# onecodex/needletail

Hardware: AMD Instinct MI355X
Metric: Gbases/s canonical k=21 on 150 bp FASTQ; % HBM-read roofline at 1/2/4/8 GPU (higher is better)
Workload: dtype u64; 1 GPU; configs[1]: synthetic FASTQ 10M x 150 bp, k=21 canonical k-mers (normalize -> reverse_complement -> canonical_kmers), reduce mode, device-resident batch; reads_total=10000000, reads_this_gpu=10000000, read_len=150, k=21, seed=0x5eed0002, outputs=n_total,n_fwd,n_rc,4096-bin prefix histogram,sum64,xor64, parallelism=single GPU, rccl_ranks=0, devices_visible=1

## Files before the change

### needletail_amd/csrc/ntk_api.hip

```cpp
#include "../../include/needletail_amd.h"

#include <hip/hip_runtime.h>
#include <rccl/rccl.h>
#include <dlfcn.h>
#include <time.h>

#include <cstdlib>
#include <cstring>
#include <map>
#include <mutex>
#include <new>
#include <utility>
#include <thread>
#include <algorithm>
#include <vector>

#include "ntk_kernels.hpp"

using namespace ntk;

const void *ntk_pick_scan2(int k, bool tie_rc, bool accept_u);
const void *ntk_pick_scan2_q(int k, bool canonical, bool tie_rc, bool accept_u);
const void *ntk_pick_scan2_min_a(int k, int w, bool tie_rc, bool accept_u, bool quality);
const void *ntk_pick_scan2_min_b(int k, int w, bool tie_rc, bool accept_u, bool quality);
const void *ntk_pick_scan2_fwd(int k, bool accept_u);

namespace {

thread_local int g_last_hip = 0;
thread_local int g_last_rccl = 0;

inline unsigned grid_for(uint64_t items, unsigned block) { const uint64_t b = (items + block - 1) / block; return (unsigned)(b > (1u << 20) ? (1u << 20) : (b ? b : 1)); }

#define HIPCHK(expr)                                     \
    do {                                                 \
        hipError_t e__ = (expr);                         \
        if (e__ != hipSuccess) {                         \
            g_last_hip = (int)e__;                       \
            (void)hipGetLastError();                     \
            return NTK_ERR_HIP;                          \
// ... 132 lines not shown
}

struct Mode { int kw; bool canon, tie_rc, accept_u; bool raw_bytes = false; };
inline uint32_t quality_cutoff(const ntk_params *p) { return (p->flags >> 8) & 0xFFu; }

int resolve_mode(const ntk_params *p, bool batch_face, Mode *m)
{
    if (!p) return NTK_ERR_BAD_ARG;
    if (p->k < 1 || p->k > (batch_face && p->path == NTK_PATH_BYTES_CANONICAL ? 255u : 32u)) return NTK_ERR_BAD_K;
    if ((p->flags & ~(0xFFFFu | NTK_FLAG_RESET)) != 0 || p->pre > NTK_PRE_NORMALIZE_IUPAC) return NTK_ERR_BAD_ARG;
    m->kw = p->k > 16 ? 2 : 1;
    m->accept_u = p->pre >= NTK_PRE_NORMALIZE;
    switch (p->path) {
    case NTK_PATH_BYTES_CANONICAL:
        m->raw_bytes = batch_face && (p->pre < NTK_PRE_NORMALIZE || p->k > 32);
        m->canon = true; m->tie_rc = true; break;
    case NTK_PATH_BITS: m->canon = false; m->tie_rc = false; break;
    case NTK_PATH_BITS_CANONICAL: m->canon = true; m->tie_rc = false; break;
    default: return NTK_ERR_BAD_ARG;
    }
    return NTK_OK;
}

constexpr int kMaxShards = 256;
constexpr uint32_t kLowerRing = 64;
constexpr uint64_t kMaxTilesPerLaunch = (uint64_t)8 << 22;

template <bool QM>
const void *pick_materialise(const Mode &m, uint32_t k)
{
#define NTK_PICK_FIX(KF, T, U)                                                                      \
    if (!QM && m.kw == 2 && m.canon && k == KF && m.tie_rc == T && m.accept_u == U)                  \
        return (const void *)&scan_kernel<2, true, T, U, false, KF>;
    NTK_PICK_FIX(21, false, false) NTK_PICK_FIX(21, false, true) NTK_PICK_FIX(21, true, true)
#undef NTK_PICK_FIX
#define NTK_PICK(KW, C, T, U)                                                                       \
    if (m.kw == KW && m.canon == C && m.tie_rc == T && m.accept_u == U)                             \
        return (const void *)&scan_kernel<KW, C, T, U, false, 0, QM>;
    NTK_PICK(1, false, false, false) NTK_PICK(1, false, false, true)
    NTK_PICK(1, true, false, false) NTK_PICK(1, true, false, true)
    NTK_PICK(1, true, true, true)
    NTK_PICK(2, false, false, false) NTK_PICK(2, false, false, true)
    NTK_PICK(2, true, false, false) NTK_PICK(2, true, false, true)
    NTK_PICK(2, true, true, true)
#undef NTK_PICK
    return nullptr;
}

const void *pick_scan(const Mode &m, uint32_t k, bool reduce, bool quality)
// ... 130 lines not shown
    if (rc) return rc;
    Fold fold;
    fold.undigested = wide;
    TimedSpan span;
    if ((rc = span.begin(c))) return rc;
    if (packed_first) {
        const FlagPair f = next_flag(c);
        launch_with_quality(c, normalized ? wide_reduce_q<true> : wide_reduce_q<false>,
                            normalized ? &wide_canonical_reduce_kernel<true> : &wide_canonical_reduce_kernel<false>, blocks, kWkThreads, d_qual, cutoff,
                            d_seq, n, p->k, c->d_part_hist, c->d_part_scalars, f.flag, f.next);
        HIPCHK(hipGetLastError());
        fold.alt_flag = f.flag; fold.alt_rows = blocks_raw;
    }
    launch_raw_bytes(c, wide, blocks_raw, d_seq, n, p->k, fold.alt_flag, normalized, d_qual, cutoff);
    HIPCHK(hipGetLastError());
    if ((rc = span.end(c->ev_used))) return rc;
    return launch_fold(c, blocks, fold);
}

struct TileScan {
    const void *fn = nullptr;
    int threads = 0;
    size_t lds = 0;
    uint32_t halo_lanes = 0;
    uint64_t max_chunk = 0;
    int max_per_cu = 0;
    bool reduce = true;
    bool speculate = false;
    uint32_t cutoff = 0;
};
inline uint64_t tile_count(uint64_t n, uint64_t tile_slots) { return ((n + 15) / 16 + tile_slots - 1) / tile_slots; }
int launch_tile_scan(ntk_ctx *c, const TileScan &s, ScanArgs &a, bool zero_first)
{
    int per_cu = 0, rc = resident_blocks(c, s.fn, s.threads, s.lds, s.max_per_cu, &per_cu);
    if (rc) return rc;
    const uint64_t blocks_max = block_cap(c, per_cu), waves_per_block = (uint64_t)s.threads / 64;
    const uint64_t tile_slots = 64 - (uint64_t)s.halo_lanes, tile_stride = tile_slots * 16, n = a.n_bytes;
    const int blocks_raw = s.speculate ? raw_bytes_blocks(c, n) : 0;
    a.n_tiles = tile_count(n, tile_slots);
    a.work_counters = c->d_work;
    a.zero_words = NTK_ACC_WORDS;
    for (uint64_t tb = 0; tb < a.n_tiles; tb += kMaxTilesPerLaunch) {
        const uint64_t te = tb + kMaxTilesPerLaunch < a.n_tiles ? tb + kMaxTilesPerLaunch : a.n_tiles;
        const uint64_t tiles = te - tb;
        uint64_t chunk = tiles / (blocks_max * waves_per_block * 4);
        chunk = chunk < 1 ? 1 : (chunk > s.max_chunk ? s.max_chunk : chunk);
        const uint64_t want_blocks = (tiles + chunk * waves_per_block - 1) / (chunk * waves_per_block);
        const int blocks = (int)(want_blocks < blocks_max ? want_blocks : blocks_max);
        a.tile_begin = tb; a.tile_end = te;
        const uint64_t first_tail = n / tile_stride;
        a.tail_tile_rel = first_tail < tb ? 0u : (first_tail - tb > 0xFFFFFFFEull ? 0xFFFFFFFFu : (uint32_t)(first_tail - tb));
        a.n_shards = blocks < kMaxShards ? (uint32_t)blocks : (uint32_t)kMaxShards;
        a.tiles_per_shard = (uint32_t)((tiles + a.n_shards - 1) / a.n_shards);
        a.chunk_tiles = (uint32_t)chunk;
        a.zero_acc = zero_first ? c->d_acc : nullptr;
        zero_first = false;
        if (c->work_dirty) HIPCHK(hipMemsetAsync(c->d_work, 0, kMaxShards * 64, c->stream));
        c->work_dirty = true;
        if (s.reduce) {
            if ((rc = ensure_partials(c, blocks > blocks_raw ? blocks : blocks_raw))) return rc;
            a.part_hist = c->d_part_hist; a.part_scalars = c->d_part_scalars;
        }
        Fold fold;
        fold.rearm_shards = a.n_shards;
        if (s.speculate) {
            const FlagPair f = next_flag(c);
            a.lower_flag = f.flag; a.lower_flag_next = f.next;
            fold.alt_flag = f.flag; fold.alt_rows = blocks_raw;
        }
        TimedSpan span;
        if ((rc = span.begin(c))) return rc;
        void *kargs[] = {(void *)&a};
        HIPCHK(hipLaunchKernel(s.fn, dim3(blocks), dim3(s.threads), kargs, s.lds, c->stream));
        if (s.speculate) {
            launch_raw_bytes(c, false, blocks_raw, a.seq, n, a.k, fold.alt_flag, false, a.qual, s.cutoff);
            HIPCHK(hipGetLastError());
        }
        if ((rc = span.end(c->ev_used))) return rc;
        if (s.reduce && (rc = launch_fold(c, blocks, fold))) return rc;
    }
    return NTK_OK;
}

int run_scan(ntk_ctx *c, const uint8_t *d_seq, uint64_t n, const ntk_params *p, const Mode &m, bool reduce,
             uint64_t *d_values, uint16_t *d_valid16, uint16_t *d_rc16, const uint8_t *d_qual = nullptr, const void *fused_min_fn = nullptr,
             int halo_lanes = kHaloLanes)
{
    const bool zero_first = reduce && (p->flags & NTK_FLAG_RESET);
    if (n == 0) {
        if (zero_first) HIPCHK(hipMemsetAsync(c->d_acc, 0, NTK_ACC_WORDS * sizeof(uint64_t), c->stream));
        return NTK_OK;
    }
    if (bad_device_input(d_seq, d_qual)) return NTK_ERR_BAD_ARG;
    const uint32_t cutoff = d_qual ? quality_cutoff(p) : 0u;
    bool speculate = false;
    if (m.raw_bytes) {
        if (p->k > 32 && (!reduce || fused_min_fn)) return NTK_ERR_BAD_K;
        if (!reduce || fused_min_fn) return NTK_ERR_UNSUPPORTED;
        const uint8_t *qual = cutoff ? d_qual : nullptr;
        speculate = p->k <= 32 && tile_count(n, 64 - (uint64_t)halo_lanes) <= kMaxTilesPerLaunch && !(c->route_off & NTK_ROUTE_NO_SPECULATION);
        if (!speculate) return run_bytes_reduce(c, d_seq, n, p, zero_first, m.accept_u, qual, cutoff);
    }
    const void *fn = fused_min_fn ? fused_min_fn : pick_scan(m, p->k, reduce, cutoff != 0);
    if (!fn) return NTK_ERR_BAD_ARG;
    int threads = !reduce ? 256 : (c->launch_threads ? c->launch_threads : 768);
    if (reduce && !c->launch_threads) {
        auto it = c->auto_threads.find(fn);
        if (it != c->auto_threads.end()) threads = it->second;
        else {
            int best_waves = 0;
            for (int t : {768, 640, 512}) {
                int blocks_cu = 0;
                HIPCHK(hipOccupancyMaxActiveBlocksPerMultiprocessor(&blocks_cu, fn, t, 0));
                if (blocks_cu > 2) blocks_cu = 2;
                if (blocks_cu * t > best_waves) { best_waves = blocks_cu * t; threads = t; }
            }
            c->auto_threads[fn] = threads;
        }
    }
    TileScan s;
    s.fn = fn; s.threads = threads; s.halo_lanes = (uint32_t)halo_lanes; s.max_chunk = 24;
    s.lds = reduce ? 0 : (size_t)(threads / 64) * kStageWaveU64 * sizeof(uint64_t);
    s.max_per_cu = reduce ? 2 * (1024 / threads) : 4;
    s.reduce = reduce; s.speculate = speculate; s.cutoff = cutoff;
    ScanArgs a;
    memset(&a, 0, sizeof(a));
    scan_args_set_k(a, p->k);
    a.seq = d_seq; a.n_bytes = n;
    a.values = d_values; a.valid16 = d_valid16; a.rc16 = d_rc16;
    scan_args_set_quality(a, d_qual, cutoff);
    return launch_tile_scan(c, s, a, zero_first);
}

const void *pick_min_generic(const Mode &m, bool quality, bool f64, uint32_t k)
{
    const int kw = f64 ? 2 : m.kw;
    const int mode = min_gen_mode(k, f64);
#define NTK_PICK_MG(KW, T, U, Q, F, MD) if (kw == KW && m.tie_rc == T && m.accept_u == U && quality == Q && f64 == F && mode == MD) return (const void *)&minimizer_scan_kernel<KW, T, U, Q, F, MD>;
#define NTK_PICK_MG3(KW, Q, F, MD) NTK_PICK_MG(KW, false, false, Q, F, MD) NTK_PICK_MG(KW, false, true, Q, F, MD) NTK_PICK_MG(KW, true, true, Q, F, MD)
#define NTK_PICK_MG6(KW, F, MD) NTK_PICK_MG3(KW, false, F, MD) NTK_PICK_MG3(KW, true, F, MD)
    NTK_PICK_MG6(2, true, 0) NTK_PICK_MG6(2, true, 1) NTK_PICK_MG6(2, true, 3) NTK_PICK_MG6(2, true, 2)
    NTK_PICK_MG6(2, false, 2)
    NTK_PICK_MG6(2, false, 1) NTK_PICK_MG6(1, false, 0) NTK_PICK_MG6(1, false, 1)
#undef NTK_PICK_MG6
#undef NTK_PICK_MG3
#undef NTK_PICK_MG
    return nullptr;
}

int run_min_scan(ntk_ctx *c, const uint8_t *d_seq, uint64_t n, const ntk_params *p, const Mode &m, uint32_t w, const uint8_t *d_qual)
{
    if (bad_device_input(d_seq, d_qual)) return NTK_ERR_BAD_ARG;
    const uint32_t cutoff = d_qual ? quality_cutoff(p) : 0u;
    const bool f64 = p->k <= 25 && !(c->route_off & NTK_ROUTE_NO_F64);
    ScanArgs a;
    memset(&a, 0, sizeof(a));
    scan_args_set_k(a, p->k);
    a.seq = d_seq; a.n_bytes = n;
    scan_args_set_quality(a, d_qual, cutoff);
    scan_args_set_window(a, w);
    TileScan s;
    s.fn = pick_min_generic(m, cutoff != 0, f64, p->k);
    if (!s.fn) return NTK_ERR_BAD_ARG;
    s.threads = min_gen_threads(f64);
    s.halo_lanes = a.min_halo_lanes; s.max_chunk = 16; s.max_per_cu = 8;
    return launch_tile_scan(c, s, a, (p->flags & NTK_FLAG_RESET) != 0);
}

void destroy_batch(ntk_batch *b)
{
    if (b->h_seq) (void)hipHostFree(b->h_seq);
    if (b->h_off) (void)hipHostFree(b->h_off);
    if (b->d_seq) (void)hipFree(b->d_seq);
    if (b->h_qual) (void)hipHostFree(b->h_qual);
    if (b->d_qual) (void)hipFree(b->d_qual);
    if (b->ev_copied) (void)hipEventDestroy(b->ev_copied);
    if (b->ev_done) (void)hipEventDestroy(b->ev_done);
    delete b;
}

int init_ctx(ntk_ctx *c, void *stream, bool borrow);

int create_ctx(int device, void *stream, bool borrow, ntk_ctx **out)
{
    if (!out) return NTK_ERR_BAD_ARG;
    *out = nullptr;
    int count = 0;
    if (hipGetDeviceCount(&count) != hipSuccess || count <= 0) { (void)hipGetLastError(); return NTK_ERR_NO_DEVICE; }
// ... 1019 lines not shown
}


static int minimizers_reduce_impl(ntk_ctx *c, const uint8_t *d_seq, const uint8_t *d_qual, uint64_t n, const ntk_params *p, uint32_t w);

int ntk_minimizers_reduce_device(ntk_ctx *c, const uint8_t *d_seq, uint64_t n, const ntk_params *p, uint32_t w)
{
    return minimizers_reduce_impl(c, d_seq, nullptr, n, p, w);
}

static int minimizers_reduce_impl(ntk_ctx *c, const uint8_t *d_seq, const uint8_t *d_qual, uint64_t n, const ntk_params *p, uint32_t w)
{
    if (!c || w < 1 || w > 256) return NTK_ERR_BAD_ARG;
    Mode m;
    int rc = resolve_mode(p, true, &m);
    if (rc) return rc;
    if (!m.canon) return NTK_ERR_BAD_ARG;
    if (m.raw_bytes) return p->k > 32 ? NTK_ERR_BAD_K : NTK_ERR_UNSUPPORTED;
    HIPCHK(hipSetDevice(c->device));
    if (n) {
        const bool masked = d_qual && quality_cutoff(p);
        const void *fn = (c->route_off & NTK_ROUTE_NO_REGFUSED) ? nullptr : pick_scan_min(m, p->k, w, masked);
        if (fn)
            return run_scan(c, d_seq, n, p, m, true, nullptr, nullptr, nullptr, masked ? d_qual : nullptr, fn, p->k + w - 1 > 32 ? 3 : 2);
        if (p->k <= 31 && w <= 49 && !(c->route_off & NTK_ROUTE_NO_GENERIC))
            return run_min_scan(c, d_seq, n, p, m, w, masked ? d_qual : nullptr);
    }
    if (p->flags & NTK_FLAG_RESET) HIPCHK(hipMemsetAsync(c->d_acc, 0, NTK_ACC_WORDS * sizeof(uint64_t), c->stream));
    if (n == 0) return NTK_OK;
    const uint64_t chunk = c->minimizer_chunk;
    const uint64_t back = (uint64_t)w + p->k - 2;
    const int blocks = c->n_cu * 4;
    if ((rc = ensure_partials(c, blocks))) return rc;
    ScanArgs a; memset(&a, 0, sizeof(a)); scan_args_set_k(a, p->k);
    for (uint64_t c0 = 0; c0 < n; c0 += chunk) {
        const uint64_t c1 = c0 + chunk < n ? c0 + chunk : n;
        const uint64_t start = c0 > back ? (c0 - back) & ~(uint64_t)15 : 0;
        const uint64_t n_sub = c1 - start, nt = (n_sub + 15) / 16 * 16;
        if ((rc = ensure_scratch(c, 3, nt * 8))) return rc;
        if ((rc = ensure_scratch(c, 4, nt / 8 + 16))) return rc;
        if ((rc = ensure_scratch(c, 5, nt / 8 + 16))) return rc;
        uint64_t *d_val = (uint64_t *)c->scratch[3].p;
        uint16_t *d_v16 = (uint16_t *)c->scratch[4].p, *d_r16 = (uint16_t *)c->scratch[5].p;
        if ((rc = run_scan(c, d_seq + start, n_sub, p, m, false, d_val, d_v16, d_r16, d_qual ? d_qual + start : nullptr))) return rc;
#define NTK_WM(WW)                                                                                                    \
    case WW:                                                                                                          \
        hipLaunchKernelGGL(window_min_reduce_kernel<WW>, dim3(blocks), dim3(kWmThreads), 0, c->stream, (const uint64_t *)d_val, \
// ... 318 lines not shown
```

### needletail_amd/csrc/ntk_kernels.hpp

```cpp
#pragma once
#include <hip/hip_runtime.h>
#include <stdint.h>
#include <type_traits>

#include "ntk_tile.hpp"

#if !defined(NTK_KBENCH) && (defined(NTK_ABL_LOADSONLY) || defined(NTK_ABL_FLOOR) || defined(NTK_ABL_NOLDS) || defined(NTK_ABL_NODIGEST) || \
                             defined(NTK_ABL_NOEXEC) || defined(NTK_ABL_NOSDWA) || defined(NTK_ABL_NOMASKALG) || defined(NTK_V_CLOCKS) || \
                             defined(NTK_X_CMPFIRST) || defined(NTK_X_TWOPHASE) || defined(NTK_X_MFMASUM) || defined(NTK_X_SELOUT) || defined(NTK_X_PREFETCH2) || defined(NTK_X_FASTSTART) || defined(NTK_ABL_HALFIMPORTS))
#error "NTK_ABL_* / NTK_X_* / NTK_V_CLOCKS are kernel-bench switches: build with -DNTK_KBENCH (tools/build_kbench.sh), never into the library"
#endif

namespace ntk {

typedef uint32_t u32x4 __attribute__((ext_vector_type(4)));

constexpr int kDppWaveShr1 = 0x138;
struct DevXL {
    __device__ __forceinline__ uint32_t prev_and(int s, uint32_t x, uint32_t mask) const { return prev(s, x) & mask; }
    __device__ __forceinline__ uint32_t prev_auto(uint32_t x) const { return prev(0, x); }
    __device__ __forceinline__ uint32_t prev(int, uint32_t x) const
    {
        return (uint32_t)__builtin_amdgcn_mov_dpp((int)x, kDppWaveShr1, 0xf, 0xf, true);
    }
    __device__ __forceinline__ uint32_t prev_add(int, uint32_t x, uint32_t c) const
    {
        uint32_t r;
        asm("s_nop 1\n v_add_u32_dpp %0, %1, %2 wave_shr:1 row_mask:0xf bank_mask:0xf bound_ctrl:1" : "=v"(r) : "v"(x), "v"(c));
        return r;
    }
    __device__ __forceinline__ uint32_t select_prev(int, bool take, uint32_t a, uint32_t b) const
    {
// ... 175 lines not shown
            uint64_t *ps = a.part_scalars + (size_t)blockIdx.x * 4;
            ps[0] = tv; ps[1] = tf; ps[2] = ts; ps[3] = tx;
        }
    }
}

template <int K, int HB>
struct DevMasks2 {
    static constexpr bool kLight = Sv2Light<K, HB>::value;
    uint64_t VA[16], VB[16];
    uint64_t sum = 0, sum2 = 0;
    uint32_t sumh = 0;
    uint32_t xh = 0, xlo = 0;
    uint32_t rep = 0;
    static constexpr int kWordCopies = K <= 6 ? (((1 << HB) >> (2 * (K <= 6 ? K : 0))) < 64 ? ((1 << HB) >> (2 * (K <= 6 ? K : 0))) : 64) : 1;
    uint32_t one = 1;
    uint32_t nf_s = 0;
    uint32_t nf_bits = 0;
#ifdef NTK_X_MFMASUM
    typedef int i32x4 __attribute__((ext_vector_type(4)));
    i32x4 macc = {0, 0, 0, 0}, msel = {0, 0, 0, 0};
#endif

    template <int KM, class Enc>
    __device__ __forceinline__ void compute(const Enc &en, bool tail_tile, int64_t lane_base, uint64_t n_bytes)
    {
        uint64_t B[16];
#ifdef NTK_X_CLEANTILE
        {
            const uint32_t dif = (en.ex[0] ^ en.uu[0]) | (en.ex[1] ^ en.uu[1]) | (en.ex[2] ^ en.uu[2]) | (en.ex[3] ^ en.uu[3]);
            if (!tail_tile && __builtin_amdgcn_ballot_w64(dif != 0u) == 0ull) {
#pragma unroll
                for (int i = 0; i < 16; i++) { VA[i] = Sv2Geom<KM>::kKeep; VB[i] = ~0ull; }
                asm volatile("" ::: "memory");
                return;
            }
        }
#endif
#ifdef NTK_ABL_NOSDWA
#pragma unroll
        for (int i = 0; i < 16; i++) B[i] = __builtin_amdgcn_ballot_w64(en.ex[i & 3] != (uint32_t)i);
        if (false) {
#endif
        NTK_SDWA_EQ(B[0], en.ex[0], en.uu[0], BYTE_0);  NTK_SDWA_EQ(B[1], en.ex[0], en.uu[0], BYTE_1);
        NTK_SDWA_EQ(B[2], en.ex[0], en.uu[0], BYTE_2);  NTK_SDWA_EQ(B[3], en.ex[0], en.uu[0], BYTE_3);
        NTK_SDWA_EQ(B[4], en.ex[1], en.uu[1], BYTE_0);  NTK_SDWA_EQ(B[5], en.ex[1], en.uu[1], BYTE_1);
        NTK_SDWA_EQ(B[6], en.ex[1], en.uu[1], BYTE_2);  NTK_SDWA_EQ(B[7], en.ex[1], en.uu[1], BYTE_3);
        NTK_SDWA_EQ(B[8], en.ex[2], en.uu[2], BYTE_0);  NTK_SDWA_EQ(B[9], en.ex[2], en.uu[2], BYTE_1);
        NTK_SDWA_EQ(B[10], en.ex[2], en.uu[2], BYTE_2); NTK_SDWA_EQ(B[11], en.ex[2], en.uu[2], BYTE_3);
        NTK_SDWA_EQ(B[12], en.ex[3], en.uu[3], BYTE_0); NTK_SDWA_EQ(B[13], en.ex[3], en.uu[3], BYTE_1);
        NTK_SDWA_EQ(B[14], en.ex[3], en.uu[3], BYTE_2); NTK_SDWA_EQ(B[15], en.ex[3], en.uu[3], BYTE_3);
#ifdef NTK_ABL_NOSDWA
        }
#endif
        if (tail_tile) {
#pragma unroll
            for (int i = 0; i < 16; i++) B[i] &= __builtin_amdgcn_ballot_w64(lane_base + i < (int64_t)n_bytes);
        }
#ifdef NTK_ABL_NOMASKALG
#pragma unroll
        for (int i = 0; i < 16; i++) { VA[i] = B[i]; VB[i] = ~0ull; }
#else
        window_masks_ab_any<KM>(B, VA, VB);
#endif
    }

    __device__ __forceinline__ uint64_t min64(uint64_t a, uint64_t b) const
    {
        uint64_t r;
        asm("v_min_f64 %0, %1, %2" : "=v"(r) : "v"(a), "v"(b));
        return r;
    }
    __device__ __forceinline__ uint32_t pk_min16_crossed(uint32_t a, uint32_t b) const
    {
        uint32_t r;
        asm("v_pk_min_u16 %0, %1, %2 op_sel:[0,1] op_sel_hi:[1,0]" : "=v"(r) : "v"(a), "v"(b));
        return r;
    }
    __device__ __forceinline__ uint32_t cell_offset_hi(uint32_t T) const
    {
        if (HB == 14) {
            uint32_t off;
            const uint32_t kMask = 0xFFFCu;
            asm("v_and_b32_sdwa %0, %1, %2 dst_sel:DWORD dst_unused:UNUSED_PAD src0_sel:DWORD src1_sel:WORD_1" : "=v"(off) : "s"(kMask), "v"(T));
            return off;
        }
// ... 289 lines not shown
#undef NTK_R_SUM_1
#undef NTK_R_SUM_0
#undef NTK_R_CNT
#undef NTK_R_CNT_FIRST
#undef NTK_R_HIST
#undef NTK_R_MASKS
#undef NTK_R_EXEC
};

struct NoSink {};

#ifndef NTK_SV2_MINWAVES
#define NTK_SV2_MINWAVES 1
#endif
template <int K, bool TIE_RC, bool ACCEPT_U, bool QM = false, int HB = 12, int W = 0, bool FWD = false>
__global__ __launch_bounds__(1024, NTK_SV2_MINWAVES) void scan2_kernel(ScanArgs a)
{
    static_assert(K >= 1 && K <= 32 && (HB == 12 || HB == 14), "sv2 covers 1 <= k <= 32");
    static_assert(W == 0 || Sv2MinFused<K, W>::value, "fused minimizers: see ntk_tile.hpp");
    static_assert(W == 0 || K <= 16 || Sv2Light<K, HB>::value, "fused minimizers sum the lo word only: the cell must cover the bits above it");
    constexpr bool WORD = K <= 16;
    constexpr bool LIGHT = Sv2Light<K, HB>::value && !WORD;
    constexpr int kCells = 1 << HB;
    using Geo = Sv2Geom<(W ? K + W - 1 : K)>;
    constexpr uint32_t kStride = Geo::kStride, kHaloB = Geo::kHaloBytes;
    struct Lds { uint32_t hist[kCells]; uint64_t red[16 * 6]; };
    __shared__ Lds L;
    uint32_t *const s_hist = L.hist;
    uint64_t *const s_red = L.red;
    if ((uint32_t)(uintptr_t)&L.hist[0] != 0u) __builtin_trap();

#ifdef NTK_V_CLOCKS
    const uint64_t dbg_c0 = clock64(), dbg_w0 = wall_clock64();
    uint32_t dbg_tiles = 0;
#endif
#ifndef NTK_X_FASTSTART
    if (a.zero_acc && blockIdx.x == 0)
        for (uint32_t i = threadIdx.x; i < a.zero_words; i += blockDim.x) a.zero_acc[i] = 0;
    for (int i = threadIdx.x; i < kCells; i += blockDim.x) s_hist[i] = 0;
    __syncthreads();

#endif
    const uint32_t lane = threadIdx.x & 63u;
    const uint32_t wave = __builtin_amdgcn_readfirstlane(threadIdx.x >> 6);
    const uint32_t shard = blockIdx.x % a.n_shards;
    const uint32_t launch_tiles = (uint32_t)(a.tile_end - a.tile_begin);
    const uint32_t shard_begin = shard * a.tiles_per_shard;
    uint32_t shard_end = shard_begin + a.tiles_per_shard;
    if (shard_end > launch_tiles) shard_end = launch_tiles;
    uint32_t *ctr = a.work_counters + shard * 16;
    const uint32_t shard_tiles = shard_begin < shard_end ? shard_end - shard_begin : 0u;
#ifdef NTK_X_FASTSTART
    uint32_t next = 0;
    if (lane == 0) next = atomicAdd(ctr, a.chunk_tiles);
    if (a.zero_acc && blockIdx.x == 0)
        for (uint32_t i = threadIdx.x; i < a.zero_words; i += blockDim.x) a.zero_acc[i] = 0;
    for (int i = threadIdx.x; i < kCells / 4; i += blockDim.x) reinterpret_cast<u32x4 *>(s_hist)[i] = u32x4{0u, 0u, 0u, 0u};
    __syncthreads();
#endif
    constexpr bool SPEC = TIE_RC && !ACCEPT_U && W == 0 && !FWD;
    uint32_t lc = 0;
    if (SPEC && a.lower_flag_next && blockIdx.x == 0 && threadIdx.x == 0) *a.lower_flag_next = 0;
    DevXL xl;
    DevMasks2<K, HB> mp;
    NoSink sink;
    mp.rep = lane & (uint32_t)(DevMasks2<K, HB>::kWordCopies - 1);
#ifdef NTK_X_MFMASUM
    { const int sel = 1 << (8 * (lane & 3)); mp.msel = {sel, sel, sel, sel}; }
#endif

#ifndef NTK_X_FASTSTART
    uint32_t next = 0;
    if (lane == 0) next = atomicAdd(ctr, a.chunk_tiles);
#endif
    next = __builtin_amdgcn_readfirstlane(next);
#ifdef NTK_X_GUIDED
    uint32_t c_cur = a.chunk_tiles;
    const uint32_t shard_waves2 = 2u * ((gridDim.x + a.n_shards - 1) / a.n_shards) * (blockDim.x >> 6);
#endif
    while (next < shard_tiles) {
        const uint32_t r0 = shard_begin + next;
#ifdef NTK_X_GUIDED
        uint32_t r1 = r0 + c_cur;
        if (r1 > shard_end) r1 = shard_end;
        {
            const uint32_t done = next + c_cur < shard_tiles ? next + c_cur : shard_tiles;
            uint32_t c = (shard_tiles - done) / shard_waves2;
            c = c < 2u ? 2u : (c > a.chunk_tiles ? a.chunk_tiles : c);
            c_cur = c;
            if (lane == 0) next = atomicAdd(ctr, c);
        }
#else
        uint32_t r1 = r0 + a.chunk_tiles;
        if (r1 > shard_end) r1 = shard_end;
        if (lane == 0) next = atomicAdd(ctr, a.chunk_tiles);
#endif
        const uint64_t t0 = a.tile_begin + r0;
// ... 29 lines not shown
#endif
        auto process = [&](const u32x4 &t, const u32x4 &q, uint32_t r, auto &&after_encode) {
            const bool tail = r >= a.tail_tile_rel;
            Raw16 raw{t.x, t.y, t.z, t.w};
            if constexpr (SPEC && !QM) {
                if (tail) lc |= or_of_input_bytes(raw, (int64_t)a.n_bytes - ((int64_t)tile_byte - (int64_t)kHaloB + lane * 16));
                else lc = bitop3<0xFE>(bitop3<0xFE>(lc, t.x, t.y), t.z, t.w);
            }
            if constexpr (QM) raw = quality_break16(raw, Raw16{q.x, q.y, q.z, q.w}, a.q_add, a.q_sel);
            if constexpr (SPEC && QM) {
                if (tail) lc |= or_of_input_bytes(lower_watch16(raw), (int64_t)a.n_bytes - ((int64_t)tile_byte - (int64_t)kHaloB + lane * 16));
                else lc = lower_watch_or(lower_watch_or(lower_watch_or(lower_watch_or(lc, raw.x), raw.y), raw.z), raw.w);
            }
#ifdef NTK_ABL_LOADSONLY
            mp.xlo ^= raw.x ^ raw.y ^ raw.z ^ raw.w; (void)tail;
            after_encode();
#elif defined(NTK_ABL_FLOOR)
            (void)tail; (void)raw;
            after_encode();
            fl_code += fl_step; fl_rcode += fl_code;
            lane_tile_sv2<TIE_RC, K>(sink, xl, mp, fl_code, fl_rcode);
#else
            const EncSV2 en = encode16_sv2<ACCEPT_U>(raw);
            mp.template compute<(W ? K + W - 1 : K)>(en, tail, (int64_t)tile_byte - (int64_t)kHaloB + lane * 16, a.n_bytes);
            after_encode();
            if constexpr (W > 0) lane_tile_sv2_min<TIE_RC, K, W>(sink, xl, mp, en.code, en.rcode);
            else if constexpr (WORD) lane_tile_sv2w<TIE_RC, K, FWD>(sink, xl, mp, en.code, en.rcode);
            else if constexpr (FWD) lane_tile_sv2_fwd<K>(sink, xl, mp, en.code);
            else lane_tile_sv2<TIE_RC, K>(sink, xl, mp, en.code, en.rcode);
#endif
            voff += kStride; tile_byte += kStride;
#ifdef NTK_V_CLOCKS
            dbg_tiles++;
#endif
        };
        u32x4 ta = load_tile(voff), qa = ta;
        if constexpr (QM) qa = load_qual(voff);
#ifdef NTK_X_PREFETCH2
        u32x4 tb = ta;
        if (r0 + 1 < r1) tb = load_tile(voff + kStride);
        for (uint32_t r = r0; r < r1; r += 2) {
            process(ta, qa, r, [&] { if (r + 2 < r1) ta = load_tile(voff + 2 * kStride); });
            if (r + 1 < r1) process(tb, qa, r + 1, [&] { if (r + 3 < r1) tb = load_tile(voff + 2 * kStride); });
        }
#else
        for (uint32_t r = r0; r < r1; r++)
            process(ta, qa, r, [&] {
                if (r + 1 < r1) { ta = load_tile(voff + kStride); if constexpr (QM) qa = load_qual(voff + kStride); }
            });
#endif
        next = __builtin_amdgcn_readfirstlane(next);
    }

#ifdef NTK_V_CLOCKS
    if ((threadIdx.x & 63) == 0 && a.values) {
        uint32_t hwid, xcc;
        asm volatile("s_getreg_b32 %0, hwreg(HW_REG_HW_ID)" : "=s"(hwid));
        asm volatile("s_getreg_b32 %0, hwreg(HW_REG_XCC_ID)" : "=s"(xcc));
        const size_t w = (size_t)blockIdx.x * (blockDim.x >> 6) + (threadIdx.x >> 6);
        a.values[w * 4 + 0] = dbg_w0; a.values[w * 4 + 1] = wall_clock64();
// ... 1221 lines not shown
```

### needletail_amd/csrc/ntk_tile.hpp

```cpp
#pragma once
#include <stdint.h>

#if defined(__HIPCC__)
#define NTK_HD __host__ __device__ __forceinline__
#else
#define NTK_HD inline
#endif

namespace ntk {

constexpr int kTileBytes = 1024;
constexpr int kHistBins = 4096;

struct ScanArgs {
    const uint8_t *seq;
    uint64_t n_bytes;
    uint64_t n_tiles;
    uint64_t tile_begin;
    uint64_t tile_end;
    uint32_t *work_counters;
    uint32_t n_shards;
    uint32_t tiles_per_shard;
    uint32_t chunk_tiles;
    uint32_t tail_tile_rel;
// ... 570 lines not shown
{
    const uint32_t mh = (uint32_t)(k.k >> 32), ml = (uint32_t)k.k;
    lo = alignbit(mh, ml, 11);
    hi = mh >> 11;
    sbit = ml & 1u;
}
NTK_HD void key_fields(KeyG k, uint32_t &lo, uint32_t &hi, uint32_t &sbit) { lo = (uint32_t)k.v; hi = (uint32_t)(k.v >> 32); sbit = k.s; }

inline void scan_args_set_window(ScanArgs &a, uint32_t w)
{
    a.min_w = w;
    a.min_halo_lanes = (uint32_t)kHaloLanes + (w - 1 + 15) / 16;
    uint32_t q = 1;
    while (2 * q <= w) q *= 2;
    a.min_overlap = w - q;
    uint32_t len = 1;
    for (int i = 0; i < 6; i++) { const uint32_t sft = len < w ? (len < w - len ? len : w - len) : 0; a.min_smear[i] = sft; len += sft; }
    const uint32_t kw = a.k + w - 1;
    len = 1;
    for (int i = 0; i < 6; i++) { const uint32_t sft = kw <= 49 && len < kw ? (len < kw - len ? len : kw - len) : 0; a.min_smear_kw[i] = sft; len += sft; }
    if (kw == 1) a.min_smear_kw[0] = 0;
}

template <int K>
NTK_HD void window_masks_ab(const uint64_t (&G)[16], uint64_t (&A)[16], uint64_t (&B)[16])
{
    static_assert(K >= 17 && K <= 32, "sv path is built for 17 <= k <= 32");
    uint64_t S[16];
    S[15] = G[15];
#pragma unroll
    for (int i = 14; i >= 0; i--) S[i] = S[i + 1] & G[i];
#pragma unroll
    for (int j = 0; j < 16; j++) {
        const int c = 17 + j - K, a_ = c > 0 ? c : 0;
        uint64_t v = S[a_] << 1;
        if (c < 0) v &= S[(33 + j - K) & 15] << 2;
        B[j] = v;
    }
#ifdef NTK_X_EXACTHALO
    A[0] = G[0];
#else
    A[0] = G[0] & ~3ull;
#endif
#pragma unroll
    for (int j = 1; j < 16; j++) A[j] = A[j - 1] & G[j];
}

template <int K>
NTK_HD void window_masks1_ab(const uint64_t (&G)[16], uint64_t (&A)[16], uint64_t (&B)[16], const uint64_t kNoHalo = ~3ull)
{
    static_assert(K >= 1 && K <= 16, "k <= 16 variant");
    constexpr uint64_t kAll = ~0ull;
    if constexpr (K >= 9) {
        uint64_t P[16], S[16], S8[8], P8[16];
        P[0] = G[0] & kNoHalo;
#pragma unroll
        for (int j = 1; j < 16; j++) P[j] = P[j - 1] & G[j];
        S[15] = G[15];
#pragma unroll
        for (int i = 14; i >= 0; i--) S[i] = S[i + 1] & G[i];
        S8[7] = G[7];
#pragma unroll
        for (int i = 6; i >= 1; i--) S8[i] = S8[i + 1] & G[i];
        P8[8] = G[8] & kNoHalo;
#pragma unroll
        for (int j = 9; j < 15; j++) P8[j] = P8[j - 1] & G[j];
// ... 9 lines not shown
    }
    constexpr int P = K >= 8 ? 8 : (K >= 4 ? 4 : (K >= 2 ? 2 : 1));
    uint64_t E[32];
#pragma unroll
    for (int i = 0; i < 16; i++) { E[16 + i] = G[i]; E[i] = G[i] << 1; }
    E[16] &= kNoHalo;
#pragma unroll
    for (int w = 1; w < P; w *= 2) {
#pragma unroll
        for (int e = 31; e >= 2 * w - 1; e--) E[e] &= E[e - w];
    }
#pragma unroll
    for (int j = 0; j < 16; j++) {
        if constexpr (K > P) {
            A[j] = E[16 + j];
            B[j] = j >= K ? (E[16 + j - (K - P)] & kNoHalo) : E[16 + j - (K - P)];
        } else {
            A[j] = E[16 + j];
            B[j] = j >= K ? kNoHalo : kAll;
        }
    }
}

template <int KM> struct Sv2Geom {
    static_assert(KM >= 1 && KM <= 48, "window of at most 48 bytes");
    static constexpr int kHalo = KM <= 32 ? 2 : 3;
    static constexpr int kSlots = 64 - kHalo;
#ifdef NTK_X_EXACTHALO
    static constexpr int kStride = (KM >= 17 && KM <= 32) ? ((1024 - (KM - 1)) & ~3) : kSlots * 16;
#else
    static constexpr int kStride = kSlots * 16;
#endif
    static constexpr int kHaloBytes = kHalo * 16;
    static constexpr uint64_t kKeep = ~((1ull << kHalo) - 1ull);
};

template <int C>
NTK_HD void window_masks_span(const uint64_t (&G)[16], uint64_t (&A)[16], uint64_t (&B)[16], uint32_t q, uint64_t keep)
{
    uint64_t S[16];
    S[15] = G[15];
#pragma unroll
    for (int i = 14; i >= 0; i--) S[i] = S[i + 1] & G[i];
    uint64_t Fq1 = ~0ull;
    for (uint32_t i = 1; i < q; i++) Fq1 &= S[0] << i;
    const uint64_t Fq = q ? (Fq1 & (S[0] << q)) : ~0ull;
#pragma unroll
    for (int j = 0; j < 16; j++) {
        if (j <= C) B[j] = (S[(15 - C + j) & 15] << (q + 1)) & Fq;
        else B[j] = (S[(j - C - 1) & 15] << q) & Fq1;
    }
    A[0] = G[0] & keep;
#pragma unroll
    for (int j = 1; j < 16; j++) A[j] = A[j - 1] & G[j];
}
template <int KM>
NTK_HD void window_masks_ab_any(const uint64_t (&G)[16], uint64_t (&A)[16], uint64_t (&B)[16])
{
    if constexpr (KM > 32) window_masks_span<(KM - 2) & 15>(G, A, B, (uint32_t)((KM - 2) >> 4), Sv2Geom<KM>::kKeep);
    else if constexpr (KM >= 17) window_masks_ab<KM>(G, A, B);
    else window_masks1_ab<KM>(G, A, B);
}
NTK_HD void window_masks_runtime(const uint64_t (&G)[16], uint64_t (&A)[16], uint64_t (&B)[16], uint32_t L, uint64_t keep)
{
    if (L >= 17) {
        const uint32_t q = (L - 2) >> 4;
        switch ((L - 2) & 15) {
#define NTK_WM_CASE(C) case C: window_masks_span<C>(G, A, B, q, keep); break;
            NTK_WM_CASE(0) NTK_WM_CASE(1) NTK_WM_CASE(2) NTK_WM_CASE(3) NTK_WM_CASE(4) NTK_WM_CASE(5) NTK_WM_CASE(6) NTK_WM_CASE(7)
            NTK_WM_CASE(8) NTK_WM_CASE(9) NTK_WM_CASE(10) NTK_WM_CASE(11) NTK_WM_CASE(12) NTK_WM_CASE(13) NTK_WM_CASE(14) NTK_WM_CASE(15)
#undef NTK_WM_CASE
        }
        return;
    }
    switch (L) {
#define NTK_WM_CASE(K) case K: window_masks1_ab<K>(G, A, B, keep); break;
        NTK_WM_CASE(1) NTK_WM_CASE(2) NTK_WM_CASE(3) NTK_WM_CASE(4) NTK_WM_CASE(5) NTK_WM_CASE(6) NTK_WM_CASE(7) NTK_WM_CASE(8)
        NTK_WM_CASE(9) NTK_WM_CASE(10) NTK_WM_CASE(11) NTK_WM_CASE(12) NTK_WM_CASE(13) NTK_WM_CASE(14) NTK_WM_CASE(15) NTK_WM_CASE(16)
#undef NTK_WM_CASE
    }
}


struct EncSV2 {
// ... 325 lines not shown
```

Before: 3312 Gbases/s.

## Use exact-halo tile stride for non-minimizer scans and promote fast-start prologue

For non-minimizer reduce scans, tiles now advance by (1024-(k-1)) rounded to 4 bytes instead of 62*16 bytes, so each tile overlaps by only k-1 bytes plus padding instead of two full 16-byte lanes. Window masks exclude the few duplicated positions, and the first tile uses split dword loads so negative offsets do not fault. This trims redundant halo reads and encode work per byte. The former fast-start prologue, which issues the work-counter atomic before zeroing the LDS histogram, becomes the default. Launch planning moves into a shared header. The change touches mask correctness at tile boundaries.

```diff
diff --git a/needletail_amd/csrc/ntk_api.hip b/needletail_amd/csrc/ntk_api.hip
--- a/needletail_amd/csrc/ntk_api.hip
+++ b/needletail_amd/csrc/ntk_api.hip
@@ -16,6 +16,7 @@
 #include <vector>
 
 #include "ntk_kernels.hpp"
+#include "ntk_plan.hpp"
 
 using namespace ntk;
 
@@ -194,9 +195,7 @@
     return NTK_OK;
 }
 
-constexpr int kMaxShards = 256;
 constexpr uint32_t kLowerRing = 64;
-constexpr uint64_t kMaxTilesPerLaunch = (uint64_t)8 << 22;
 
 template <bool QM>
 const void *pick_materialise(const Mode &m, uint32_t k)
@@ -373,37 +372,31 @@
     const void *fn = nullptr;
     int threads = 0;
     size_t lds = 0;
-    uint32_t halo_lanes = 0;
+    uint32_t stride = 0;
     uint64_t max_chunk = 0;
     int max_per_cu = 0;
     bool reduce = true;
     bool speculate = false;
     uint32_t cutoff = 0;
 };
-inline uint64_t tile_count(uint64_t n, uint64_t tile_slots) { return ((n + 15) / 16 + tile_slots - 1) / tile_slots; }
 int launch_tile_scan(ntk_ctx *c, const TileScan &s, ScanArgs &a, bool zero_first)
 {
     int per_cu = 0, rc = resident_blocks(c, s.fn, s.threads, s.lds, s.max_per_cu, &per_cu);
     if (rc) return rc;
     const uint64_t blocks_max = block_cap(c, per_cu), waves_per_block = (uint64_t)s.threads / 64;
-    const uint64_t tile_slots = 64 - (uint64_t)s.halo_lanes, tile_stride = tile_slots * 16, n = a.n_bytes;
+    const uint64_t n = a.n_bytes;
     const int blocks_raw = s.speculate ? raw_bytes_blocks(c, n) : 0;
-    a.n_tiles = tile_count(n, tile_slots);
+    a.n_tiles = tile_count(n, s.stride);
     a.work_counters = c->d_work;
     a.zero_words = NTK_ACC_WORDS;
     for (uint64_t tb = 0; tb < a.n_tiles; tb += kMaxTilesPerLaunch) {
-        const uint64_t te = tb + kMaxTilesPerLaunch < a.n_tiles ? tb + kMaxTilesPerLaunch : a.n_tiles;
-        const uint64_t tiles = te - tb;
-        uint64_t chunk = tiles / (blocks_max * waves_per_block * 4);
-        chunk = chunk < 1 ? 1 : (chunk > s.max_chunk ? s.max_chunk : chunk);
-        const uint64_t want_blocks = (tiles + chunk * waves_per_block - 1) / (chunk * waves_per_block);
-        const int blocks = (int)(want_blocks < blocks_max ? want_blocks : blocks_max);
-        a.tile_begin = tb; a.tile_end = te;
-        const uint64_t first_tail = n / tile_stride;
-        a.tail_tile_rel = first_tail < tb ? 0u : (first_tail - tb > 0xFFFFFFFEull ? 0xFFFFFFFFu : (uint32_t)(first_tail - tb));
-        a.n_shards = blocks < kMaxShards ? (uint32_t)blocks : (uint32_t)kMaxShards;
-        a.tiles_per_shard = (uint32_t)((tiles + a.n_shards - 1) / a.n_shards);
-        a.chunk_tiles = (uint32_t)chunk;
+        const LaunchPlan lp = plan_launch(n, s.stride, tb, blocks_max, waves_per_block, s.max_chunk);
+        const int blocks = (int)lp.blocks;
+        a.tile_begin = lp.tile_begin; a.tile_end = lp.tile_end;
+        a.tail_tile_rel = lp.tail_tile_rel;
+        a.n_shards = lp.n_shards;
+        a.tiles_per_shard = lp.tiles_per_shard;
+        a.chunk_tiles = lp.chunk_tiles;
         a.zero_acc = zero_first ? c->d_acc : nullptr;
         zero_first = false;
         if (c->work_dirty) HIPCHK(hipMemsetAsync(c->d_work, 0, kMaxShards * 64, c->stream));
@@ -435,7 +428,7 @@
 
 int run_scan(ntk_ctx *c, const uint8_t *d_seq, uint64_t n, const ntk_params *p, const Mode &m, bool reduce,
              uint64_t *d_values, uint16_t *d_valid16, uint16_t *d_rc16, const uint8_t *d_qual = nullptr, const void *fused_min_fn = nullptr,
-             int halo_lanes = kHaloLanes)
+             uint32_t fused_w = 0)
 {
     const bool zero_first = reduce && (p->flags & NTK_FLAG_RESET);
     if (n == 0) {
@@ -444,12 +437,13 @@
     }
     if (bad_device_input(d_seq, d_qual)) return NTK_ERR_BAD_ARG;
     const uint32_t cutoff = d_qual ? quality_cutoff(p) : 0u;
+    const uint32_t stride = !reduce ? (uint32_t)kTileStride : (p->k <= 32 ? (uint32_t)sv2_stride_bytes((int)(fused_w ? p->k + fused_w - 1 : p->k), fused_w == 0) : 0u);
     bool speculate = false;
     if (m.raw_bytes) {
         if (p->k > 32 && (!reduce || fused_min_fn)) return NTK_ERR_BAD_K;
         if (!reduce || fused_min_fn) return NTK_ERR_UNSUPPORTED;
         const uint8_t *qual = cutoff ? d_qual : nullptr;
-        speculate = p->k <= 32 && tile_count(n, 64 - (uint64_t)halo_lanes) <= kMaxTilesPerLaunch && !(c->route_off & NTK_ROUTE_NO_SPECULATION);
+        speculate = p->k <= 32 && tile_count(n, stride) <= kMaxTilesPerLaunch && !(c->route_off & NTK_ROUTE_NO_SPECULATION);
         if (!speculate) return run_bytes_reduce(c, d_seq, n, p, zero_first, m.accept_u, qual, cutoff);
     }
     const void *fn = fused_min_fn ? fused_min_fn : pick_scan(m, p->k, reduce, cutoff != 0);
@@ -470,7 +464,7 @@
         }
     }
     TileScan s;
-    s.fn = fn; s.threads = threads; s.halo_lanes = (uint32_t)halo_lanes; s.max_chunk = 24;
+    s.fn = fn; s.threads = threads; s.stride = stride; s.max_chunk = 24;
     s.lds = reduce ? 0 : (size_t)(threads / 64) * kStageWaveU64 * sizeof(uint64_t);
     s.max_per_cu = reduce ? 2 * (1024 / threads) : 4;
     s.reduce = reduce; s.speculate = speculate; s.cutoff = cutoff;
@@ -514,7 +508,7 @@
     s.fn = pick_min_generic(m, cutoff != 0, f64, p->k);
     if (!s.fn) return NTK_ERR_BAD_ARG;
     s.threads = min_gen_threads(f64);
-    s.halo_lanes = a.min_halo_lanes; s.max_chunk = 16; s.max_per_cu = 8;
+    s.stride = (64u - a.min_halo_lanes) * 16u; s.max_chunk = 16; s.max_per_cu = 8;
     return launch_tile_scan(c, s, a, (p->flags & NTK_FLAG_RESET) != 0);
 }
 
@@ -1580,7 +1574,7 @@
         const bool masked = d_qual && quality_cutoff(p);
         const void *fn = (c->route_off & NTK_ROUTE_NO_REGFUSED) ? nullptr : pick_scan_min(m, p->k, w, masked);
         if (fn)
-            return run_scan(c, d_seq, n, p, m, true, nullptr, nullptr, nullptr, masked ? d_qual : nullptr, fn, p->k + w - 1 > 32 ? 3 : 2);
+            return run_scan(c, d_seq, n, p, m, true, nullptr, nullptr, nullptr, masked ? d_qual : nullptr, fn, w);
         if (p->k <= 31 && w <= 49 && !(c->route_off & NTK_ROUTE_NO_GENERIC))
             return run_min_scan(c, d_seq, n, p, m, w, masked ? d_qual : nullptr);
     }
diff --git a/needletail_amd/csrc/ntk_kernels.hpp b/needletail_amd/csrc/ntk_kernels.hpp
--- a/needletail_amd/csrc/ntk_kernels.hpp
+++ b/needletail_amd/csrc/ntk_kernels.hpp
@@ -7,7 +7,7 @@
 
 #if !defined(NTK_KBENCH) && (defined(NTK_ABL_LOADSONLY) || defined(NTK_ABL_FLOOR) || defined(NTK_ABL_NOLDS) || defined(NTK_ABL_NODIGEST) || \
                              defined(NTK_ABL_NOEXEC) || defined(NTK_ABL_NOSDWA) || defined(NTK_ABL_NOMASKALG) || defined(NTK_V_CLOCKS) || \
-                             defined(NTK_X_CMPFIRST) || defined(NTK_X_TWOPHASE) || defined(NTK_X_MFMASUM) || defined(NTK_X_SELOUT) || defined(NTK_X_PREFETCH2) || defined(NTK_X_FASTSTART) || defined(NTK_ABL_HALFIMPORTS))
+                             defined(NTK_X_CMPFIRST) || defined(NTK_X_TWOPHASE) || defined(NTK_X_MFMASUM) || defined(NTK_X_SELOUT) || defined(NTK_X_PREFETCH2) || defined(NTK_ABL_HALFIMPORTS))
 #error "NTK_ABL_* / NTK_X_* / NTK_V_CLOCKS are kernel-bench switches: build with -DNTK_KBENCH (tools/build_kbench.sh), never into the library"
 #endif
 
@@ -229,21 +229,10 @@
     i32x4 macc = {0, 0, 0, 0}, msel = {0, 0, 0, 0};
 #endif
 
-    template <int KM, class Enc>
+    template <int KM, bool EXACT, class Enc>
     __device__ __forceinline__ void compute(const Enc &en, bool tail_tile, int64_t lane_base, uint64_t n_bytes)
     {
         uint64_t B[16];
-#ifdef NTK_X_CLEANTILE
-        {
-            const uint32_t dif = (en.ex[0] ^ en.uu[0]) | (en.ex[1] ^ en.uu[1]) | (en.ex[2] ^ en.uu[2]) | (en.ex[3] ^ en.uu[3]);
-            if (!tail_tile && __builtin_amdgcn_ballot_w64(dif != 0u) == 0ull) {
-#pragma unroll
-                for (int i = 0; i < 16; i++) { VA[i] = Sv2Geom<KM>::kKeep; VB[i] = ~0ull; }
-                asm volatile("" ::: "memory");
-                return;
-            }
-        }
-#endif
 #ifdef NTK_ABL_NOSDWA
 #pragma unroll
         for (int i = 0; i < 16; i++) B[i] = __builtin_amdgcn_ballot_w64(en.ex[i & 3] != (uint32_t)i);
@@ -268,7 +257,7 @@
 #pragma unroll
         for (int i = 0; i < 16; i++) { VA[i] = B[i]; VB[i] = ~0ull; }
 #else
-        window_masks_ab_any<KM>(B, VA, VB);
+        window_masks_ab_any<KM, EXACT>(B, VA, VB);
 #endif
     }
 
@@ -604,7 +593,7 @@
     constexpr bool WORD = K <= 16;
     constexpr bool LIGHT = Sv2Light<K, HB>::value && !WORD;
     constexpr int kCells = 1 << HB;
-    using Geo = Sv2Geom<(W ? K + W - 1 : K)>;
+    using Geo = Sv2Geom<(W ? K + W - 1 : K), (W == 0)>;
     constexpr uint32_t kStride = Geo::kStride, kHaloB = Geo::kHaloBytes;
     struct Lds { uint32_t hist[kCells]; uint64_t red[16 * 6]; };
     __shared__ Lds L;
@@ -615,13 +604,6 @@
 #ifdef NTK_V_CLOCKS
     const uint64_t dbg_c0 = clock64(), dbg_w0 = wall_clock64();
     uint32_t dbg_tiles = 0;
-#endif
-#ifndef NTK_X_FASTSTART
-    if (a.zero_acc && blockIdx.x == 0)
-        for (uint32_t i = threadIdx.x; i < a.zero_words; i += blockDim.x) a.zero_acc[i] = 0;
-    for (int i = threadIdx.x; i < kCells; i += blockDim.x) s_hist[i] = 0;
-    __syncthreads();
-
 #endif
     const uint32_t lane = threadIdx.x & 63u;
     const uint32_t wave = __builtin_amdgcn_readfirstlane(threadIdx.x >> 6);
@@ -632,14 +614,12 @@
     if (shard_end > launch_tiles) shard_end = launch_tiles;
     uint32_t *ctr = a.work_counters + shard * 16;
     const uint32_t shard_tiles = shard_begin < shard_end ? shard_end - shard_begin : 0u;
-#ifdef NTK_X_FASTSTART
     uint32_t next = 0;
     if (lane == 0) next = atomicAdd(ctr, a.chunk_tiles);
     if (a.zero_acc && blockIdx.x == 0)
         for (uint32_t i = threadIdx.x; i < a.zero_words; i += blockDim.x) a.zero_acc[i] = 0;
     for (int i = threadIdx.x; i < kCells / 4; i += blockDim.x) reinterpret_cast<u32x4 *>(s_hist)[i] = u32x4{0u, 0u, 0u, 0u};
     __syncthreads();
-#endif
     constexpr bool SPEC = TIE_RC && !ACCEPT_U && W == 0 && !FWD;
     uint32_t lc = 0;
     if (SPEC && a.lower_flag_next && blockIdx.x == 0 && threadIdx.x == 0) *a.lower_flag_next = 0;
@@ -651,10 +631,6 @@
     { const int sel = 1 << (8 * (lane & 3)); mp.msel = {sel, sel, sel, sel}; }
 #endif
 
-#ifndef NTK_X_FASTSTART
-    uint32_t next = 0;
-    if (lane == 0) next = atomicAdd(ctr, a.chunk_tiles);
-#endif
     next = __builtin_amdgcn_readfirstlane(next);
 #ifdef NTK_X_GUIDED
     uint32_t c_cur = a.chunk_tiles;
@@ -730,7 +706,7 @@
             lane_tile_sv2<TIE_RC, K>(sink, xl, mp, fl_code, fl_rcode);
 #else
             const EncSV2 en = encode16_sv2<ACCEPT_U>(raw);
-            mp.template compute<(W ? K + W - 1 : K)>(en, tail, (int64_t)tile_byte - (int64_t)kHaloB + lane * 16, a.n_bytes);
+            mp.template compute<(W ? K + W - 1 : K), (W == 0)>(en, tail, (int64_t)tile_byte - (int64_t)kHaloB + lane * 16, a.n_bytes);
             after_encode();
             if constexpr (W > 0) lane_tile_sv2_min<TIE_RC, K, W>(sink, xl, mp, en.code, en.rcode);
             else if constexpr (WORD) lane_tile_sv2w<TIE_RC, K, FWD>(sink, xl, mp, en.code, en.rcode);
@@ -742,8 +718,19 @@
             dbg_tiles++;
 #endif
         };
-        u32x4 ta = load_tile(voff), qa = ta;
-        if constexpr (QM) qa = load_qual(voff);
+        auto load_first = [&](__amdgpu_buffer_rsrc_t r_, uint32_t off) {
+            uint32_t d[4];
+#pragma unroll
+            for (int i = 0; i < 4; i++) {
+                const int32_t o = (int32_t)off + 4 * i;
+                const uint32_t v = __builtin_amdgcn_raw_buffer_load_b32(r_, o >= 0 ? (uint32_t)o : 0u, 0, 0);
+                d[i] = o >= 0 ? v : 0u;
+            }
+            return u32x4{d[0], d[1], d[2], d[3]};
+        };
+        const bool split_first = kHaloB % 16u != 0u && t0 == 0;
+        u32x4 ta = split_first ? load_first(rs, voff) : load_tile(voff), qa = ta;
+        if constexpr (QM) qa = split_first ? load_first(rq, voff) : load_qual(voff);
 #ifdef NTK_X_PREFETCH2
         u32x4 tb = ta;
         if (r0 + 1 < r1) tb = load_tile(voff + kStride);
diff --git a/needletail_amd/csrc/ntk_plan.hpp b/needletail_amd/csrc/ntk_plan.hpp
--- /dev/null
+++ b/needletail_amd/csrc/ntk_plan.hpp
@@ -0,0 +1,39 @@
+#pragma once
+#include <stdint.h>
+
+namespace ntk {
+
+constexpr int kMaxShards = 256;
+constexpr uint64_t kMaxTilesPerLaunch = (uint64_t)8 << 22;
+
+inline uint64_t tile_count(uint64_t n, uint64_t stride) { return (n + stride - 1) / stride; }
+
+struct LaunchPlan {
+    uint64_t tile_begin, tile_end;
+    uint32_t chunk_tiles;
+    uint32_t blocks;
+    uint32_t n_shards;
+    uint32_t tiles_per_shard;
+    uint32_t tail_tile_rel;
+};
+
+inline LaunchPlan plan_launch(uint64_t n, uint64_t stride, uint64_t tile_begin, uint64_t blocks_max, uint64_t waves_per_block, uint64_t max_chunk)
+{
+    LaunchPlan p;
+    const uint64_t n_tiles = tile_count(n, stride);
+    p.tile_begin = tile_begin;
+    p.tile_end = tile_begin + kMaxTilesPerLaunch < n_tiles ? tile_begin + kMaxTilesPerLaunch : n_tiles;
+    const uint64_t tiles = p.tile_end - p.tile_begin;
+    uint64_t chunk = tiles / (blocks_max * waves_per_block * 4);
+    chunk = chunk < 1 ? 1 : (chunk > max_chunk ? max_chunk : chunk);
+    const uint64_t want_blocks = (tiles + chunk * waves_per_block - 1) / (chunk * waves_per_block);
+    p.blocks = (uint32_t)(want_blocks < blocks_max ? want_blocks : blocks_max);
+    p.chunk_tiles = (uint32_t)chunk;
+    p.n_shards = p.blocks < (uint32_t)kMaxShards ? (p.blocks ? p.blocks : 1u) : (uint32_t)kMaxShards;
+    p.tiles_per_shard = (uint32_t)((tiles + p.n_shards - 1) / p.n_shards);
+    const uint64_t first_tail = n / stride;
+    p.tail_tile_rel = first_tail < tile_begin ? 0u : (first_tail - tile_begin > 0xFFFFFFFEull ? 0xFFFFFFFFu : (uint32_t)(first_tail - tile_begin));
+    return p;
+}
+
+}
diff --git a/needletail_amd/csrc/ntk_tile.hpp b/needletail_amd/csrc/ntk_tile.hpp
--- a/needletail_amd/csrc/ntk_tile.hpp
+++ b/needletail_amd/csrc/ntk_tile.hpp
@@ -616,10 +616,16 @@
     if (kw == 1) a.min_smear_kw[0] = 0;
 }
 
-template <int K>
+constexpr int sv2_stride_bytes(int km, bool exact)
+{
+    return km > 32 ? 61 * 16 : (!exact ? 62 * 16 : (km <= 16 ? 63 * 16 : ((kTileBytes - (km - 1)) & ~3)));
+}
+template <int K, bool EXACT = false>
 NTK_HD void window_masks_ab(const uint64_t (&G)[16], uint64_t (&A)[16], uint64_t (&B)[16])
 {
     static_assert(K >= 17 && K <= 32, "sv path is built for 17 <= k <= 32");
+    constexpr int kOverlap = EXACT ? kTileBytes - sv2_stride_bytes(K, true) - (K - 1) : 0;
+    static_assert(kOverlap >= 0 && K - 17 + kOverlap <= 16, "the overlap windows end in lane 1");
     uint64_t S[16];
     S[15] = G[15];
 #pragma unroll
@@ -629,13 +635,10 @@
         const int c = 17 + j - K, a_ = c > 0 ? c : 0;
         uint64_t v = S[a_] << 1;
         if (c < 0) v &= S[(33 + j - K) & 15] << 2;
+        if (c >= 0 && c < kOverlap) v &= ~2ull;
         B[j] = v;
     }
-#ifdef NTK_X_EXACTHALO
-    A[0] = G[0];
-#else
-    A[0] = G[0] & ~3ull;
-#endif
+    A[0] = EXACT ? G[0] : G[0] & ~3ull;
 #pragma unroll
     for (int j = 1; j < 16; j++) A[j] = A[j - 1] & G[j];
 }
@@ -691,17 +694,15 @@
     }
 }
 
-template <int KM> struct Sv2Geom {
+template <int KM, bool EXACT = false> struct Sv2Geom {
     static_assert(KM >= 1 && KM <= 48, "window of at most 48 bytes");
-    static constexpr int kHalo = KM <= 32 ? 2 : 3;
+    static constexpr int kHalo = KM > 32 ? 3 : ((!EXACT || KM >= 17) ? 2 : 1);
     static constexpr int kSlots = 64 - kHalo;
-#ifdef NTK_X_EXACTHALO
-    static constexpr int kStride = (KM >= 17 && KM <= 32) ? ((1024 - (KM - 1)) & ~3) : kSlots * 16;
-#else
-    static constexpr int kStride = kSlots * 16;
-#endif
-    static constexpr int kHaloBytes = kHalo * 16;
+    static constexpr int kStride = sv2_stride_bytes(KM, EXACT);
+    static constexpr int kHaloBytes = kTileBytes - kStride;
+    static constexpr int kOverlap = (EXACT && KM >= 17 && KM <= 32) ? kHaloBytes - (KM - 1) : 0;
     static constexpr uint64_t kKeep = ~((1ull << kHalo) - 1ull);
+    static_assert(kStride % 4 == 0 && kOverlap >= 0 && kOverlap <= 3 && kSlots * 16 <= kStride, "tile geometry");
 };
 
 template <int C>
@@ -723,12 +724,12 @@
 #pragma unroll
     for (int j = 1; j < 16; j++) A[j] = A[j - 1] & G[j];
 }
-template <int KM>
+template <int KM, bool EXACT = false>
 NTK_HD void window_masks_ab_any(const uint64_t (&G)[16], uint64_t (&A)[16], uint64_t (&B)[16])
 {
-    if constexpr (KM > 32) window_masks_span<(KM - 2) & 15>(G, A, B, (uint32_t)((KM - 2) >> 4), Sv2Geom<KM>::kKeep);
-    else if constexpr (KM >= 17) window_masks_ab<KM>(G, A, B);
-    else window_masks1_ab<KM>(G, A, B);
+    if constexpr (KM > 32) window_masks_span<(KM - 2) & 15>(G, A, B, (uint32_t)((KM - 2) >> 4), Sv2Geom<KM, false>::kKeep);
+    else if constexpr (KM >= 17) window_masks_ab<KM, EXACT>(G, A, B);
+    else window_masks1_ab<KM>(G, A, B, Sv2Geom<KM, EXACT>::kKeep);
 }
 NTK_HD void window_masks_runtime(const uint64_t (&G)[16], uint64_t (&A)[16], uint64_t (&B)[16], uint32_t L, uint64_t keep)
 {
```

New measurement: 3366 Gbases/s (median of 6 runs). 1.02x the previous value.
